# wenhao728/VORTA

Measured on AMD Instinct MI355X. Metric: video_tokens_per_sec (routed-attention denoising step, HunyuanVideo 720p 129f), higher is better.
Workload: dtype fp16

## Files before the change

vorta_amd/_debug.py:

```python
import os

KEYS = ("coreset_kv_order", "fused_text_splits", "sta_merge", "fp8_center_k", "joint_projection", "attn_variant", "no_xcd_remap",
        "sp_staging", "sp_group_streams", "sp_v_wire", "sp_emulate_link_gbps")


def _parse(text: str) -> dict:
    out = {}
    for item in filter(None, (x.strip() for x in text.split(","))):
        key, _, value = item.partition("=")
        if key not in KEYS:
            raise ValueError(f"VORTA_DEBUG: unknown key {key!r} (one of {KEYS})")
        out[key] = value if value else "1"
    return out


FLAGS = _parse(os.environ.get("VORTA_DEBUG", ""))


def flag(key: str, default: str) -> str:
    if key not in KEYS:
        raise KeyError(key)
    return FLAGS.get(key, default)
```

vorta_amd/csrc/attn_common.h:

```cpp
#pragma once
#include <hip/hip_runtime.h>
#include <stdint.h>

#include "vorta_hip.h"
#include "common.h"

namespace vorta_attn {


constexpr int KVB = 64;
constexpr int D = 128;
constexpr int ROWB = D * 2;
constexpr int TILE_BYTES = KVB * ROWB;
constexpr int BUF_BYTES = 2 * TILE_BYTES;

struct Params {
  const char* q; const char* k; const char* v; char* o;
  int64_t q_sh, k_sh, v_sh, o_sh;
  int64_t q_ss, k_ss, v_ss, o_ss;
  const int32_t* head_list; const int32_t* n_heads_dev;
  int n_heads;
  int n_q, q_group_len, q_row_offset, q_valid;
  int n_groups, blocks_per_group;
  const int32_t* q_rows; int64_t q_rows_sh;
  int n_kv, kv_row_offset;
  const int32_t* n_kv_dev; const int32_t* q_valid_dev;
  const int32_t* kv_rows; int64_t kv_rows_sh, kv_rows_sg;
  const int32_t* dup_rows; int64_t dup_rows_sh; int n_dup_pos, n_dup;
  float scale_log2;
  int n_splits, blocks_per_split;
  float* ws_o; float* ws_ml;
  int xcd_remap;
  float defer_log2;
  const int32_t* q_block_table;
  int wg_per_slot;
};

__device__ __forceinline__ void q_block_of(const Params& p, int qb, int rows_per_block, int& grp, int& p0, int& pend) {
  if (p.q_block_table) {
    const int32_t* t = p.q_block_table + 3 * qb;
    grp = t[0]; p0 = t[1]; pend = t[2];
  } else {
    grp = qb / p.blocks_per_group;
    p0 = grp * p.q_group_len + (qb - grp * p.blocks_per_group) * rows_per_block;
    pend = min((grp + 1) * p.q_group_len, p.n_q);
  }
}

__device__ __forceinline__ int live_order(const Params& p, int b, int n, bool remap) {
  if (p.n_heads_dev) n = min(n, max(*p.n_heads_dev, 0) * p.wg_per_slot);
  if (!remap || b >= n) return b;
  const int xcd = b & 7, qd = n >> 3, r = n & 7;
  return (xcd < r ? xcd * (qd + 1) : r * (qd + 1) + (xcd - r) * qd) + (b >> 3);
}

#ifndef VORTA_MAX_SEGMENTS
#define VORTA_MAX_SEGMENTS VORTA_MAX_FUSED_LAUNCHES
#endif
constexpr int MAX_SEGMENTS = VORTA_MAX_SEGMENTS;
template <class PP> __host__ __device__ __forceinline__ Params& base_of(PP& pp) { return pp.p; }
template <class PP> __host__ __device__ __forceinline__ const Params& base_of(const PP& pp) { return pp.p; }
__host__ __device__ __forceinline__ Params& base_of(Params& p) { return p; }
__host__ __device__ __forceinline__ const Params& base_of(const Params& p) { return p; }

template <class PP> struct MultiOf {
  PP seg[MAX_SEGMENTS];
  int start[MAX_SEGMENTS + 1];
  int n;
};

template <class PP>
__device__ __forceinline__ const PP& segment_of(const MultiOf<PP>& mp, int b, int& wg) {
  int s = 0;
#pragma unroll
  for (int i = 1; i < MAX_SEGMENTS; ++i) s += (i < mp.n && b >= mp.start[i]) ? 1 : 0;
  wg = live_order(base_of(mp.seg[s]), b - mp.start[s], mp.start[s + 1] - mp.start[s], true);
  return mp.seg[s];
}

__device__ __forceinline__ float2 out_descale(const Params&, int, int) { return make_float2(1.f, 1.f); }
template <class PP> __device__ __forceinline__ float2 out_descale(const PP& pp, int head, int lane) {
  return *(const float2*)(pp.v_descale + (int64_t)head * pp.v_descale_sh + lane * 2);
}

template <typename T, class PP>
__global__ __launch_bounds__(256) void attn_combine_kernel(const PP pp) {
  const Params& p = base_of(pp);
  const int lane = threadIdx.x & 63;
  const int64_t item = (int64_t)blockIdx.x * 4 + (threadIdx.x >> 6);
  if (item >= (int64_t)p.n_heads * p.n_q) return;
  const int y = (int)(item / p.n_q);
  const int pos = (int)(item - (int64_t)y * p.n_q);
  if (p.n_heads_dev && y >= *p.n_heads_dev) return;
  const int head = p.head_list ? p.head_list[y] : y;
  float m = -1e30f;
  for (int s = 0; s < p.n_splits; ++s) m = fmaxf(m, p.ws_ml[(((int64_t)y * p.n_splits + s) * p.n_q + pos) * 2]);
  float acc0 = 0.f, acc1 = 0.f, l = 0.f;
  for (int s = 0; s < p.n_splits; ++s) {
    const int64_t slot = ((int64_t)y * p.n_splits + s) * p.n_q + pos;
    const float w = __builtin_amdgcn_exp2f(p.ws_ml[slot * 2] - m);
    l += w * p.ws_ml[slot * 2 + 1];
// ... 28 lines not shown

template <typename T, class PP>
int launch_single(void (*kernel)(PP), int block_rows, const PP& pp, hipStream_t st) {
  const Params& p = base_of(pp);
  const int64_t total = (int64_t)p.n_groups * p.blocks_per_group * p.n_heads * p.n_splits;
  if (total <= 0) return VORTA_OK;
  if (total > 0x7fffffff) return VORTA_EINVAL;
  hipLaunchKernelGGL(kernel, dim3((unsigned)total), dim3(block_rows * 2), 0, st, pp);
  const hipError_t e = hipGetLastError();
  if (e != hipSuccess) return vorta_set_hip_error(e);
  return launch_combine<T>(pp, st);
}

template <class F>
int fwd_single(const F& f, const vorta_attn_args* a, void* hip_stream) {
  typename F::PP pp{};
  int block_rows = 0;
  const int rc = f.fill(a, pp, block_rows);
  if (rc != VORTA_OK) return rc;
  if (base_of(pp).n_heads == 0 || base_of(pp).n_groups == 0) return VORTA_OK;
  hipStream_t st = (hipStream_t)hip_stream;
  if (f.out_dtype(*a) == VORTA_BF16) return launch_single<__bf16>(F::template kernel<__bf16>(*a, pp, block_rows), block_rows, pp, st);
  return launch_single<_Float16>(F::template kernel<_Float16>(*a, pp, block_rows), block_rows, pp, st);
}

template <typename T, class PP>
int launch_fused(void (*kernel)(MultiOf<PP>), const MultiOf<PP>& mp, int total, hipStream_t st) {
  hipLaunchKernelGGL(kernel, dim3((unsigned)total), dim3(512), 0, st, mp);
  const hipError_t e = hipGetLastError();
  if (e != hipSuccess) return vorta_set_hip_error(e);
  for (int i = 0; i < mp.n; ++i) {
    const int rc = launch_combine<T>(mp.seg[i], st);
    if (rc != VORTA_OK) return rc;
  }
  return VORTA_OK;
}

template <class F>
int fwd_batch(const F& f, const vorta_attn_args* args, int32_t n, void* hip_stream) {
  if (!args || n < 0 || n > MAX_SEGMENTS) return VORTA_EINVAL;
  MultiOf<typename F::PP> mp{};
  int64_t total = 0;
  int dtype = -1, m = 0;
  for (int i = 0; i < n; ++i) {
    typename F::PP pp{};
    int block_rows = 0;
    const int rc = f.fill(&args[i], pp, block_rows);
    if (rc != VORTA_OK) return rc;
    Params& p = base_of(pp);
    if (p.n_heads == 0 || p.n_groups == 0) continue;
    if (block_rows != 256 || !f.fusable(args[i], pp)) return VORTA_EUNSUPPORTED;
    if (dtype >= 0 && dtype != f.out_dtype(args[i])) return VORTA_EINVAL;
    dtype = f.out_dtype(args[i]);
    p.xcd_remap = 0;
    mp.seg[m] = pp;
    mp.start[m] = (int)total;
    total += (int64_t)p.n_groups * p.blocks_per_group * p.n_heads * p.n_splits;
    if (total > 0x7fffffff) return VORTA_EINVAL;
    ++m;
  }
  if (m == 0) return VORTA_OK;
  for (int i = m; i <= MAX_SEGMENTS; ++i) mp.start[i] = (int)total;
  mp.n = m;
  hipStream_t st = (hipStream_t)hip_stream;
  if (dtype == VORTA_BF16) return launch_fused<__bf16>(F::template multi<__bf16>, mp, (int)total, st);
  return launch_fused<_Float16>(F::template multi<_Float16>, mp, (int)total, st);
}

int fill_params(const vorta_attn_args* a, Params& p, int& block_rows, int in_esize, int v_esize = 0, int k_esize = 0);
int mx_fwd(const vorta_attn_args* a, const vorta_attn_fp8_ext* ext, void* hip_stream);
int mx_fwd_batch(const vorta_attn_args* args, const vorta_attn_fp8_ext* ext, int32_t n, void* hip_stream);

template <typename T> struct MF;
template <> struct MF<__bf16> {
  using v8 = bf16x8; using v4 = bf16x4;
  static __device__ __forceinline__ f32x16 mfma(v8 a, v8 b, f32x16 c) {
    return __builtin_amdgcn_mfma_f32_32x32x16_bf16(a, b, c, 0, 0, 0);
  }
  static __device__ __forceinline__ v4 tr(const char* p) {
    return __builtin_amdgcn_ds_read_tr16_b64_v4bf16((LDS_AS v4*)p);
  }
};
template <> struct MF<_Float16> {
  using v8 = f16x8; using v4 = f16x4;
  static __device__ __forceinline__ f32x16 mfma(v8 a, v8 b, f32x16 c) {
    return __builtin_amdgcn_mfma_f32_32x32x16_f16(a, b, c, 0, 0, 0);
  }
  static __device__ __forceinline__ v4 tr(const char* p) {
    typedef __attribute__((ext_vector_type(4))) __fp16 h4;
    h4 r = __builtin_amdgcn_ds_read_tr16_b64_v4f16((LDS_AS h4*)p);
    return *(v4*)&r;
  }
};

__device__ __forceinline__ float half_max(float x) {
  auto r = __builtin_amdgcn_permlane32_swap(__float_as_uint(x), __float_as_uint(x), false, false);
  return fmaxf(__uint_as_float(r[0]), __uint_as_float(r[1]));
}
__device__ __forceinline__ float half_sum(float x) {
// ... 7 lines not shown
```

vorta_amd/csrc/attn_fwd.hip:

```cpp
#include <hip/hip_runtime.h>
#include <stdint.h>

#include "vorta_hip.h"
#include "common.h"

#include "attn_common.h"
#include "attn_fwd_diag.inc"

namespace {
using namespace vorta_attn;

template <typename T, int NW>
__global__ __launch_bounds__(NW * 64, 2) void attn_fwd_kernel(const Params p) {
  using V8 = typename MF<T>::v8;
  using V4 = typename MF<T>::v4;
  constexpr int NT = NW * 64;
  constexpr int QB = NW * 32;
  constexpr int CH = (KVB * 16) / NT;
  constexpr int ROWSTEP = NT / 16;

  __shared__ __attribute__((aligned(16))) char smem[2 * BUF_BYTES];

  const int wg = live_order(p, blockIdx.x, gridDim.x, p.xcd_remap);
  const int sp = wg % p.n_splits;
  const int rest = wg / p.n_splits;
  const int n_qb = p.n_groups * p.blocks_per_group;
  const int qb = rest % n_qb;
  const int y = rest / n_qb;
  if (p.n_heads_dev && y >= *p.n_heads_dev) return;
  const int head = p.head_list ? p.head_list[y] : y;
  int grp, p0, pend;
  q_block_of(p, qb, QB, grp, p0, pend);

  const int tid = threadIdx.x;
// ... 181 lines not shown
      }
    }
    return;
  }
  if (!row_ok) return;
  const float inv = (my_p < q_valid && l_tot > 0.f) ? 1.f / l_tot : 0.f;
  uint2 packed[16];
#pragma unroll
  for (int dt = 0; dt < 4; ++dt)
#pragma unroll
    for (int rg = 0; rg < 4; ++rg) {
      V4 t;
#pragma unroll
      for (int j = 0; j < 4; ++j) t[j] = (T)(o[dt][4 * rg + j] * inv);
      packed[dt * 4 + rg] = *(uint2*)&t;
    }
  char* obase = p.o + (int64_t)head * p.o_sh + hh * 8;
  auto store_row = [&](int64_t row) {
    char* op = obase + row * p.o_ss;
#pragma unroll
    for (int dt = 0; dt < 4; ++dt)
#pragma unroll
      for (int rg = 0; rg < 4; ++rg) *(uint2*)(op + (32 * dt + 8 * rg) * 2) = packed[dt * 4 + rg];
  };
  store_row(my_row);
  if (p.dup_rows && my_p < p.n_dup_pos) {
    const int32_t* dr = p.dup_rows + (int64_t)y * p.dup_rows_sh + (int64_t)my_p * p.n_dup;
    for (int i = 0; i < p.n_dup; ++i) store_row((int64_t)dr[i]);
  }
}

constexpr int RING = 2;

template <typename T, int NW, bool KVTAB, int NS>
__device__ __forceinline__ void attn_pipe_dma_body(const Params& p, char* __restrict__ smem, const int wg) {
  static_assert(NS == 2, "ring depth");
  TRACE_ENTRY_()
  using V8 = typename MF<T>::v8;
  using V4 = typename MF<T>::v4;
  constexpr int NT = NW * 64;
  constexpr int QB = NW * 32;
  constexpr int CH = (KVB * 16) / NT;
  constexpr int ROWSTEP = NT / 16;
#ifndef VORTA_KPRE
#define VORTA_KPRE 2
#endif
  constexpr int KPRE = (NW == 4 && KVTAB && VORTA_KPRE > 1) ? 1 : VORTA_KPRE;
  const int sp = wg % p.n_splits;
  const int rest = wg / p.n_splits;
  const int n_qb = p.n_groups * p.blocks_per_group;
  const int qb = rest % n_qb;
  const int y = rest / n_qb;
  if (p.n_heads_dev && y >= *p.n_heads_dev) return;
  const int head = p.head_list ? p.head_list[y] : y;
  int grp, p0, pend;
  q_block_of(p, qb, QB, grp, p0, pend);

  const int tid = threadIdx.x;
  const int lane = tid & 63;
  const int wave = __builtin_amdgcn_readfirstlane(tid >> 6);
  const int r32 = lane & 31;
  const int hh = lane >> 5;

  const int n_kv = p.n_kv_dev ? max(1, min(*p.n_kv_dev, p.n_kv)) : p.n_kv;
  const int q_valid = p.q_valid_dev ? min(*p.q_valid_dev, p.q_valid) : p.q_valid;
  const int nblk_total = (n_kv + KVB - 1) / KVB;
  const int blk0 = sp * p.blocks_per_split;
  const int blk1 = min(blk0 + p.blocks_per_split, nblk_total);

  const int wrow0 = p0 + wave * 32;
  const bool wave_active = wrow0 < pend;
  const int my_p = wrow0 + r32;
  const int ld_p = min(my_p, pend - 1);
  const int32_t* q_rows = p.q_rows ? p.q_rows + (int64_t)y * p.q_rows_sh : nullptr;
  const int64_t my_row = q_rows ? (int64_t)q_rows[ld_p] : (int64_t)(p.q_row_offset + ld_p);

  V8 qf[8];
  {
    const char* qp = p.q + (int64_t)head * p.q_sh + my_row * p.q_ss + hh * 16;
#pragma unroll
    for (int ks = 0; ks < 8; ++ks) {
      const V8 raw = *(const V8*)(qp + ks * 32);
#pragma unroll
      for (int i = 0; i < 8; ++i) qf[ks][i] = (T)((float)raw[i] * p.scale_log2);
    }
  }

  const int32_t* kv_rows =
      p.kv_rows ? p.kv_rows + (int64_t)y * p.kv_rows_sh + (int64_t)grp * p.kv_rows_sg : nullptr;
  const char* kbase = p.k + (int64_t)head * p.k_sh + (tid & 15) * 16;
  const char* vbase = p.v + (int64_t)head * p.v_sh + (tid & 15) * 16;
  const int lrow0 = tid >> 4;
  const int lcc = tid & 15;
  const __amdgpu_buffer_rsrc_t k_rsrc = __builtin_amdgcn_make_buffer_rsrc(
      (void*)(p.k + (int64_t)head * p.k_sh), 0, 0x7fffffff, 0x00020000);
  const __amdgpu_buffer_rsrc_t v_rsrc = __builtin_amdgcn_make_buffer_rsrc(
      (void*)(p.v + (int64_t)head * p.v_sh), 0, 0x7fffffff, 0x00020000);
  const int k_ss32 = (int)p.k_ss, v_ss32 = (int)p.v_ss;
// ... 5 lines not shown
    v_col[i] = ((lane & 15) ^ ((row & 3) << 2)) << 4;
  }
  int rowK[CH], rowV[CH];
  int posK[CH];
  unsigned offK[CH], offV[CH];
  const unsigned k_step = (unsigned)(KVB * k_ss32), v_step = (unsigned)(KVB * v_ss32);
#define ROWS_OF(dst_, blk_, clamp_)                                               \
  _Pragma("unroll") for (int i_ = 0; i_ < CH; ++i_) {                             \
    int pos_ = (blk_) * KVB + 4 * (CH * wave + i_) + (lane >> 4);                 \
    if constexpr (clamp_) pos_ = min(pos_, n_kv - 1);                             \
    if constexpr (KVTAB) dst_[i_] = kv_rows[pos_];                                \
    else dst_[i_] = p.kv_row_offset + pos_;                                       \
  }
#define K_OFF(i_) ((int)__umul24((unsigned)rowK[i_], (unsigned)k_ss32) + k_col[i_])
#define V_OFF(i_) ((int)__umul24((unsigned)rowV[i_], (unsigned)v_ss32) + v_col[i_])
#define DMA_K_AT(par_, off_) _Pragma("unroll") for (int i_ = 0; i_ < CH; ++i_) __builtin_amdgcn_raw_ptr_buffer_load_lds( \
      k_rsrc, (LDS_AS void*)(smem + (par_) * TILE_BYTES + (CH * wave + i_) * 1024), 16, (int)(off_), 0, 0, 0);
#define DMA_V_AT(par_, off_) _Pragma("unroll") for (int i_ = 0; i_ < CH; ++i_) __builtin_amdgcn_raw_ptr_buffer_load_lds( \
      v_rsrc, (LDS_AS void*)(smem + (NS + (par_)) * TILE_BYTES + (CH * wave + i_) * 1024), 16, (int)(off_), 0, 0, 0);
#define DMA_K(par_) DMA_K_AT(par_, K_OFF(i_))
#define DMA_V(par_) DMA_V_AT(par_, V_OFF(i_))

  int k_rd[8];
#pragma unroll
  for (int ks = 0; ks < 8; ++ks) k_rd[ks] = r32 * ROWB + (((2 * ks + hh) ^ (r32 & 15)) << 4);
  int v_rd[4];
  {
    const int g = lane >> 4, i16 = lane & 15, q4 = i16 >> 2, pp = i16 & 3;
#pragma unroll
    for (int dt = 0; dt < 4; ++dt)
      v_rd[dt] = NS * TILE_BYTES + (4 * (g >> 1) + q4) * ROWB + ((dt ^ q4) << 6) + 32 * (g & 1) + 8 * pp;
  }

  f32x16 o[4];
#pragma unroll
  for (int dt = 0; dt < 4; ++dt)
#pragma unroll
    for (int i = 0; i < 16; ++i) o[dt][i] = 0.f;
  float m_run = -1e30f, l_run = 0.f;
  const float defer = p.defer_log2;
  f32x16 sA0, sA1, sB0, sB1;
  f32x16 minit;
#pragma unroll
  for (int i = 0; i < 16; ++i) minit[i] = 0.f;
  float mx_cur = -1e30f;

#define QK(d0_, d1_, par_)                                                        \
  {                                                                               \
    _Pragma("unroll") for (int ks_ = 0; ks_ < 8; ++ks_) {                         \
      const V8 k0_ = *(const V8*)(smem + (par_) * TILE_BYTES + k_rd[ks_]);        \
      const V8 k1_ = *(const V8*)(smem + (par_) * TILE_BYTES + k_rd[ks_] + 32 * ROWB); \
      d0_ = MF<T>::mfma(k0_, qf[ks_], ks_ == 0 ? minit : d0_);                    \
      d1_ = MF<T>::mfma(k1_, qf[ks_], ks_ == 0 ? minit : d1_);                    \
    }                                                                             \
  }
#define ROW_MAX(dst_, a_, b_)                                                      \
  {                                                                               \
    float mx_ = a_[0];                                                            \
    _Pragma("unroll") for (int i_ = 1; i_ < 16; ++i_) mx_ = fmaxf(mx_, a_[i_]);   \
    _Pragma("unroll") for (int i_ = 0; i_ < 16; ++i_) mx_ = fmaxf(mx_, b_[i_]);   \
    dst_ = half_max(mx_);                                                         \
  }
#define ROW_MAX_POS(dst_, a_, b_)                                                  \
  {                                                                               \
    int m0_ = max(max(__float_as_int(a_[0]), __float_as_int(a_[1])), __float_as_int(a_[2])); \
    int m1_ = max(max(__float_as_int(b_[0]), __float_as_int(b_[1])), __float_as_int(b_[2])); \
    _Pragma("unroll") for (int i_ = 3; i_ < 15; i_ += 2) {                        \
      m0_ = max(max(m0_, __float_as_int(a_[i_])), __float_as_int(a_[i_ + 1]));    \
      m1_ = max(max(m1_, __float_as_int(b_[i_])), __float_as_int(b_[i_ + 1]));    \
    }                                                                             \
    m0_ = max(max(m0_, __float_as_int(a_[15])), __float_as_int(b_[15]));          \
    m0_ = max(m0_, m1_);                                                          \
    auto r_ = __builtin_amdgcn_permlane32_swap((unsigned)m0_, (unsigned)m0_, false, false); \
    dst_ = __int_as_float(max((int)r_[0], (int)r_[1]));                           \
  }
#define QK_PRE(d0_, d1_, par_)                                                    \
  {                                                                               \
// ... 52 lines not shown
  _Pragma("unroll") for (int g_ = 0; g_ < 16; ++g_) {                             \
    __builtin_amdgcn_sched_group_barrier(0x008, 1, 0);                            \
    __builtin_amdgcn_sched_group_barrier(0x100, 1, 0);                            \
    __builtin_amdgcn_sched_group_barrier(0x400, 2, 0);                            \
    __builtin_amdgcn_sched_group_barrier(0x002, 2, 0);                            \
  }                                                                               \
  _Pragma("unroll") for (int g_ = 0; g_ < 16; ++g_) {                             \
    __builtin_amdgcn_sched_group_barrier(0x008, 1, 0);                            \
    __builtin_amdgcn_sched_group_barrier(0x100, 2, 0);                            \
    __builtin_amdgcn_sched_group_barrier(0x002, 4, 0);                            \
  }
#else
#define SCHED_RECIPE()
#endif
#define STEP(c0_, c1_, n0_, n1_, kcur_, knext_, vfree_, j_, tail_)                \
  {  \
    STAGE_DMA(kcur_, vfree_, j_, tail_)                                           \
    STEP_BODY(c0_, c1_, n0_, n1_, kcur_, knext_, j_, tail_)                       \
    STEP_SYNC()                                                                   \
  }
#define STEP_BODY(c0_, c1_, n0_, n1_, kcur_, knext_, j_, tail_)                   \
  {                                                                               \
    if (wave_active) {                                                            \
      V8 kpre_[KPRE > 0 ? KPRE : 1][2];                                                          \
      _Pragma("unroll") for (int ks_ = 0; ks_ < KPRE; ++ks_) {                    \
        kpre_[ks_][0] = *(const V8*)(smem + (knext_) * TILE_BYTES + k_rd[ks_]);   \
        kpre_[ks_][1] = *(const V8*)(smem + (knext_) * TILE_BYTES + k_rd[ks_] + 32 * ROWB); \
      }                                                                           \
       \
       \
      if ((tail_) && (j_) * KVB + KVB > n_kv) {                                   \
        int h4_ = 4 * hh;  \
        asm volatile("" : "+v"(h4_));                                             \
        _Pragma("unroll") for (int i_ = 0; i_ < 16; ++i_) {                       \
          const int row_ = (i_ & 3) + 8 * (i_ >> 2) + h4_;                        \
          if ((j_) * KVB + row_ >= n_kv) c0_[i_] = -INFINITY;                     \
          if ((j_) * KVB + 32 + row_ >= n_kv) c1_[i_] = -INFINITY;                \
        }                                                                         \
        ROW_MAX(mx_cur, c0_, c1_)                                                 \
      }                                                                           \
       \
       \
       \
      if (!__all(mx_cur <= defer)) {                                              \
        const float g_ = fmaxf(mx_cur, 0.f);                                      \
        RAISE_REF(g_, c0_, c1_)                                                   \
      }                                                                           \
      V8 pb_[4];                                                                  \
      QK_PRE(n0_, n1_, knext_)     \
      float lsum_ = 0.f;                                                          \
      _Pragma("unroll") for (int i_ = 0; i_ < 16; ++i_) {                         \
        c0_[i_] = __builtin_amdgcn_exp2f(c0_[i_]);                                \
        c1_[i_] = __builtin_amdgcn_exp2f(c1_[i_]);                                \
        lsum_ += c0_[i_] + c1_[i_];                                               \
      }                                                                           \
      l_run += lsum_;                                                             \
      _Pragma("unroll") for (int e_ = 0; e_ < 8; ++e_) {                          \
        pb_[0][e_] = (T)c0_[e_];                                                  \
        pb_[1][e_] = (T)c0_[8 + e_];                                              \
        pb_[2][e_] = (T)c1_[e_];                                                  \
        pb_[3][e_] = (T)c1_[8 + e_];                                              \
      }                                                                           \
      _Pragma("unroll") for (int dt_ = 0; dt_ < 4; ++dt_) {                       \
        _Pragma("unroll") for (int kg_ = 0; kg_ < 4; ++kg_) {                     \
          const V4 lo_ = MF<T>::tr(smem + (kcur_) * TILE_BYTES + v_rd[dt_] + (16 * kg_) * ROWB); \
          const V4 hi_ = MF<T>::tr(smem + (kcur_) * TILE_BYTES + v_rd[dt_] + (16 * kg_ + 8) * ROWB); \
          V8 vf_;                                                                 \
          _Pragma("unroll") for (int e_ = 0; e_ < 4; ++e_) { vf_[e_] = lo_[e_]; vf_[4 + e_] = hi_[e_]; } \
          o[dt_] = MF<T>::mfma(vf_, pb_[kg_], o[dt_]);                            \
        }                                                                         \
      }                                                                           \
      ROW_MAX_POS(mx_cur, n0_, n1_)  \
      SCHED_RECIPE()                                                              \
    }                                                                             \
  }

  if (blk0 < blk1) {
    ROWS_OF(rowK, blk0, true)
    _Pragma("unroll") for (int i_ = 0; i_ < CH; ++i_) rowV[i_] = rowK[i_];
    DMA_K(0)
    DMA_V(0)
    ROWS_OF(rowK, blk0 + 1, true)
    DMA_K(1)
    _Pragma("unroll") for (int i_ = 0; i_ < CH; ++i_) rowV[i_] = rowK[i_];
    ROWS_OF(rowK, blk0 + NS, true)
    _Pragma("unroll") for (int i_ = 0; i_ < CH; ++i_) posK[i_] = (blk0 + NS) * KVB + 4 * (CH * wave + i_) + (lane >> 4);
    if constexpr (!KVTAB) {
      _Pragma("unroll") for (int i_ = 0; i_ < CH; ++i_) { offK[i_] = (unsigned)K_OFF(i_); offV[i_] = (unsigned)V_OFF(i_); }
    }
    __syncthreads();
    if (wave_active) {
      QK(sA0, sA1, 0)
      if (blk0 * KVB + KVB > n_kv) {
#pragma unroll
        for (int i = 0; i < 16; ++i) {
          const int row = (i & 3) + 8 * (i >> 2) + 4 * hh;
          if (blk0 * KVB + row >= n_kv) sA0[i] = -INFINITY;
          if (blk0 * KVB + 32 + row >= n_kv) sA1[i] = -INFINITY;
        }
      }
      ROW_MAX(mx_cur, sA0, sA1)
      m_run = mx_cur;
#pragma unroll
      for (int i = 0; i < 16; ++i) { sA0[i] -= m_run; sA1[i] -= m_run; minit[i] = -m_run; }
      asm volatile("" : "+v"(minit));
      mx_cur = 0.f;
    }
    __syncthreads();
  }
  const int blk_whole = min(blk1, n_kv / KVB - (KVTAB ? NS + 1 : NS));
  int blk = blk0;
  for (; blk + 1 < blk_whole; blk += 2) {
    STEP(sA0, sA1, sB0, sB1, 0, 1, 1, blk, false)
    STEP(sB0, sB1, sA0, sA1, 1, 0, 0, blk + 1, false)
  }
  if constexpr (!KVTAB) {
    if (blk > blk0 && blk < blk1) {
      ROWS_OF(rowV, blk + 1, true)
      ROWS_OF(rowK, blk + NS, true)
      _Pragma("unroll") for (int i_ = 0; i_ < CH; ++i_) posK[i_] = (blk + NS) * KVB + 4 * (CH * wave + i_) + (lane >> 4);
    }
  }
  for (; blk < blk1; blk += 2) {
    STEP(sA0, sA1, sB0, sB1, 0, 1, 1, blk, true)
    if (blk + 1 >= blk1) break;
    STEP(sB0, sB1, sA0, sA1, 1, 0, 0, blk + 1, true)
  }
#undef QK
#undef QK_PRE
#undef ROW_MAX
#undef ROW_MAX_POS
#undef RAISE_REF
#undef STEP
#undef STEP_BODY
#undef STAGE_DMA
#undef STEP_SYNC
#undef ROWS_OF
#undef DMA_K
#undef DMA_V
#undef DMA_K_AT
#undef DMA_V_AT
#undef K_OFF
#undef V_OFF

  TRACE_FLUSH_()
  if (!wave_active) return;
  int tid_e = threadIdx.x;
  asm volatile("" : "+v"(tid_e));
  const int hh_e = (tid_e >> 5) & 1;
  const int e_p = wrow0 + (tid_e & 31);
  const bool e_ok = e_p < pend;
  const int64_t e_row = q_rows ? (int64_t)q_rows[min(e_p, pend - 1)] : (int64_t)(p.q_row_offset + min(e_p, pend - 1));
  const float l_tot = half_sum(l_run);
  if (p.n_splits > 1) {
    if (e_ok) {
      const int64_t slot = ((int64_t)y * p.n_splits + sp) * p.n_q + e_p;
      float* wo = p.ws_o + slot * D;
#pragma unroll
      for (int dt = 0; dt < 4; ++dt)
#pragma unroll
        for (int rg = 0; rg < 4; ++rg) {
          f32x4 v = {o[dt][4 * rg], o[dt][4 * rg + 1], o[dt][4 * rg + 2], o[dt][4 * rg + 3]};
          *(f32x4*)(wo + 32 * dt + 8 * rg + 4 * hh_e) = v;
        }
      if (hh_e == 0) {
        p.ws_ml[slot * 2] = m_run;
        p.ws_ml[slot * 2 + 1] = l_tot;
      }
    }
    return;
  }
  if (!e_ok) return;
  const float inv = (e_p < q_valid && l_tot > 0.f) ? 1.f / l_tot : 0.f;
  uint2 packed[16];
#pragma unroll
  for (int dt = 0; dt < 4; ++dt)
#pragma unroll
    for (int rg = 0; rg < 4; ++rg) {
      V4 t;
#pragma unroll
      for (int j = 0; j < 4; ++j) t[j] = (T)(o[dt][4 * rg + j] * inv);
      packed[dt * 4 + rg] = *(uint2*)&t;
    }
  char* obase = p.o + (int64_t)head * p.o_sh + hh_e * 8;
  auto store_row = [&](int64_t row) {
    char* op = obase + row * p.o_ss;
#pragma unroll
    for (int dt = 0; dt < 4; ++dt)
#pragma unroll
      for (int rg = 0; rg < 4; ++rg) *(uint2*)(op + (32 * dt + 8 * rg) * 2) = packed[dt * 4 + rg];
  };
  store_row(e_row);
  if (p.dup_rows && e_p < p.n_dup_pos) {
    const int32_t* dr = p.dup_rows + (int64_t)y * p.dup_rows_sh + (int64_t)e_p * p.n_dup;
    for (int i = 0; i < p.n_dup; ++i) store_row((int64_t)dr[i]);
  }
}


template <typename T, int NW, bool KVTAB>
__global__ __launch_bounds__(NW * 64, 2) void attn_fwd_pipe_kernel(const Params p) {
#if defined(__HIP_DEVICE_COMPILE__)
  constexpr int NS = RING;
  __shared__ __attribute__((aligned(16))) char smem[2 * NS * TILE_BYTES];
  const int wg = live_order(p, blockIdx.x, gridDim.x, p.xcd_remap);
  attn_pipe_dma_body<T, NW, KVTAB, NS>(p, smem, wg);
#endif
}


template <typename T>
__global__ __launch_bounds__(512, 2) void attn_fwd_multi_kernel(const MultiOf<Params> mp) {
#if defined(__HIP_DEVICE_COMPILE__)
  __shared__ __attribute__((aligned(16))) char smem[2 * RING * TILE_BYTES];
  int wg;
  const Params& p = segment_of(mp, blockIdx.x, wg);
  if (p.kv_rows) attn_pipe_dma_body<T, 8, true, RING>(p, smem, wg);
  else attn_pipe_dma_body<T, 8, false, RING>(p, smem, wg);
#endif
}

}

int vorta_attn::fill_params(const vorta_attn_args* a, Params& p, int& block_rows, int in_esize, int v_esize, int k_esize) {
  if (v_esize == 0) v_esize = in_esize;
  if (k_esize == 0) k_esize = in_esize;
  if (!a || a->struct_size != sizeof(vorta_attn_args)) return VORTA_EINVAL;
  if (in_esize == 2 ? (a->dtype != VORTA_BF16 && a->dtype != VORTA_FP16) : a->dtype != VORTA_FP8E4M3) return VORTA_EUNSUPPORTED;
  if (a->head_dim != D) return VORTA_EUNSUPPORTED;
  if (a->n_heads < 0 || a->n_q < 0 || a->n_kv < 0) return VORTA_EINVAL;
  if (a->n_heads == 0 || a->n_q == 0) { block_rows = 0; p.n_groups = 0; p.blocks_per_group = 0; p.n_heads = 0; return VORTA_OK; }
  if (a->n_kv == 0) return VORTA_EINVAL;
  if (!a->q.ptr || !a->k.ptr || !a->v.ptr || !a->o.ptr) return VORTA_EINVAL;
  const vorta_tensor* ts[4] = {&a->q, &a->k, &a->v, &a->o};
  for (int i = 0; i < 4; ++i) {
    const vorta_tensor* t = ts[i];
    const int al = 16 / (i == 0 ? in_esize : i == 1 ? k_esize : i == 2 ? v_esize : 2);
    if (((uintptr_t)t->ptr & 15) || (t->stride_s % al) || (t->stride_h % al) || t->stride_s < D) return VORTA_EINVAL;
  }
  if (a->n_splits < 1 || a->n_splits > 1024) return VORTA_EINVAL;
  if (!(a->scale > 0.f)) return VORTA_EINVAL;
  if (a->n_splits > 1 && (!a->ws_o || !a->ws_ml)) return VORTA_EINVAL;
  if (a->q_group_len < 0 || a->q_valid < 0) return VORTA_EINVAL;
  if (a->dup_rows && (a->n_dup < 0 || a->n_dup_pos < 0 || a->n_dup_pos > a->n_q)) return VORTA_EINVAL;
  if (a->block_rows != 0 && a->block_rows != 128 && a->block_rows != 256) return VORTA_EINVAL;
  if (a->variant < 0 || a->variant > 2) return VORTA_EINVAL;
  if (a->variant != 1 && (a->k.stride_s * k_esize >= (1 << 24) || a->v.stride_s * v_esize >= (1 << 24))) return VORTA_EUNSUPPORTED;
  if (a->variant != 1 && !a->kv_rows) {
    const int64_t last = (int64_t)a->kv_row_offset + a->n_kv;
    const int64_t ks = a->k.stride_s * k_esize, vs = a->v.stride_s * v_esize;
    const int64_t ss = ks > vs ? ks : vs;
// ... 4 lines not shown
  p.q_ss = a->q.stride_s * in_esize; p.k_ss = a->k.stride_s * k_esize; p.v_ss = a->v.stride_s * v_esize; p.o_ss = a->o.stride_s * 2;
  p.head_list = a->head_list; p.n_heads_dev = a->n_heads_dev; p.n_heads = a->n_heads;
  p.n_q = a->n_q; p.q_group_len = a->q_group_len > 0 ? a->q_group_len : a->n_q;
  p.q_row_offset = a->q_row_offset; p.q_valid = a->q_valid;
  p.q_rows = a->q_rows; p.q_rows_sh = a->q_rows_stride_h;
  p.n_kv = a->n_kv; p.kv_row_offset = a->kv_row_offset;
  p.n_kv_dev = a->n_kv_dev; p.q_valid_dev = a->q_valid_dev;
  p.kv_rows = a->kv_rows; p.kv_rows_sh = a->kv_rows_stride_h; p.kv_rows_sg = a->kv_rows_stride_g;
  p.dup_rows = a->dup_rows; p.dup_rows_sh = a->dup_rows_stride_h; p.n_dup_pos = a->n_dup_pos; p.n_dup = a->n_dup;
  p.scale_log2 = a->scale * 1.4426950408889634f;
  p.n_splits = a->n_splits; p.ws_o = a->ws_o; p.ws_ml = a->ws_ml;
  p.xcd_remap = (a->reserved & 1) ? 0 : 1;
  p.defer_log2 = (a->reserved & 4) ? 0.f : 6.f;
  p.n_groups = (p.n_q + p.q_group_len - 1) / p.q_group_len;
  block_rows = a->block_rows;
  if (block_rows == 0) {
    const int g = p.q_group_len;
    const int64_t pad256 = ((g + 255) / 256) * 256, pad128 = ((g + 127) / 128) * 128;
    block_rows = (pad256 * 100 > pad128 * 106) ? 128 : 256;
  }
  p.blocks_per_group = (p.q_group_len + block_rows - 1) / block_rows;
  p.q_block_table = a->q_block_table;
  if (a->q_block_table) {
    if (a->n_q_blocks <= 0 || (a->block_rows != 128 && a->block_rows != 256)) return VORTA_EINVAL;
    p.n_groups = a->n_q_blocks;
    p.blocks_per_group = 1;
  }
  const int nblk = (p.n_kv + KVB - 1) / KVB;
  p.blocks_per_split = (nblk + p.n_splits - 1) / p.n_splits;
  p.wg_per_slot = p.n_groups * p.blocks_per_group * p.n_splits;
  return VORTA_OK;
}

namespace {
using namespace vorta_attn;

struct Family16 {
  using PP = Params;
  int fill(const vorta_attn_args* a, Params& p, int& block_rows) const { return fill_params(a, p, block_rows, 2); }
  bool fusable(const vorta_attn_args& a, const Params&) const { return a.variant != 1; }
  int out_dtype(const vorta_attn_args& a) const { return a.dtype; }
  template <typename T> static constexpr auto multi = attn_fwd_multi_kernel<T>;
  template <typename T> static auto kernel(const vorta_attn_args& a, const Params& p, int block_rows) {
    if (a.variant == 1) return block_rows == 256 ? attn_fwd_kernel<T, 8> : attn_fwd_kernel<T, 4>;
    if (block_rows == 256) return p.kv_rows ? attn_fwd_pipe_kernel<T, 8, true> : attn_fwd_pipe_kernel<T, 8, false>;
    return p.kv_rows ? attn_fwd_pipe_kernel<T, 4, true> : attn_fwd_pipe_kernel<T, 4, false>;
  }
};
}

extern "C" int vorta_attn_workspace_bytes(const vorta_attn_args* a, uint64_t* ws_o_bytes, uint64_t* ws_ml_bytes) {
  if (!a || a->struct_size != sizeof(vorta_attn_args) || !ws_o_bytes || !ws_ml_bytes) return VORTA_EINVAL;
  if (a->n_splits <= 1) { *ws_o_bytes = 0; *ws_ml_bytes = 0; return VORTA_OK; }
  const uint64_t slots = (uint64_t)a->n_heads * (uint64_t)a->n_splits * (uint64_t)a->n_q;
  *ws_o_bytes = slots * D * sizeof(float);
  *ws_ml_bytes = slots * 2 * sizeof(float);
  return VORTA_OK;
}

extern "C" int vorta_attn_plan(const vorta_attn_args* a, int32_t* block_rows_out, int64_t* n_workgroups_out,
                               int32_t* kernel_id_out) {
  Params p{};
  int block_rows = 0;
  int rc = vorta_attn::fill_params(a, p, block_rows, (a && a->dtype == VORTA_FP8E4M3) ? 1 : 2);
  if (rc != VORTA_OK) return rc;
  if (block_rows_out) *block_rows_out = block_rows;
  if (kernel_id_out) {
    const bool pipe = a->variant != 1;
    *kernel_id_out = (block_rows == 256 ? 8 : 4) * 16 + (pipe ? 1 : 0) + ((pipe && a->kv_rows) ? 2 : 0);
  }
  if (n_workgroups_out) *n_workgroups_out = (int64_t)p.n_groups * p.blocks_per_group * p.n_heads * (p.n_heads ? p.n_splits : 0);
  return VORTA_OK;
}

// ... 6 lines not shown
```

vorta_amd/ops.py:

```python
from __future__ import annotations

import ctypes as C
import math
from typing import NamedTuple, Optional, Sequence, Tuple

import torch

from . import _C

_DT = {torch.bfloat16: _C.VORTA_BF16, torch.float16: _C.VORTA_FP16}
FP8_STORAGE = torch.uint8


class Timeline:

    def __init__(self):
        self.records = []

    def summary(self):
        torch.cuda.synchronize()
        out = {}
        for tag, br, nwg, flops, e0, e1 in self.records:
            d = out.setdefault((tag, br), dict(launches=0, ms=0.0, flops=0.0, workgroups=0))
            d["launches"] += 1
            d["ms"] += e0.elapsed_time(e1)
            d["flops"] += flops
            d["workgroups"] += nwg
        return out


_timeline: Optional[Timeline] = None
from ._debug import flag as _debug_flag
DEFAULT_VARIANT = int(_debug_flag("attn_variant", "0"))
NO_XCD_REMAP = int(_debug_flag("no_xcd_remap", "0"))


def set_timeline(t: Optional[Timeline]):
    global _timeline
    _timeline = t


def _stream() -> int:
    return torch.cuda.current_stream().cuda_stream


def _require_gpu(*ts: torch.Tensor):
    for t in ts:
        if t is not None and not t.is_cuda:
            raise _C.VortaHipError("vorta_amd ops need tensors on an MI355X (cuda) device; there is no CPU path")


def _tensor(t: torch.Tensor) -> _C.Tensor:
    if t.dim() != 3 or t.stride(2) != 1:
        raise ValueError(f"expected a (H,S,D) view with contiguous D, got shape {tuple(t.shape)} strides {t.stride()}")
    return _C.Tensor(t.data_ptr(), t.stride(0), t.stride(1))


def _ptr(t: Optional[torch.Tensor], dtype=torch.int32):
    if t is None:
        return None
    if t.dtype != dtype or not t.is_contiguous():
        raise ValueError(f"index tables must be contiguous {dtype}")
    return t.data_ptr()


def fold_heads(x: torch.Tensor) -> torch.Tensor:
    if x.dim() == 3:
# ... 105 lines not shown
            raise ValueError("query groups need kv_rows_stride_g (one key list per group)")
        elif kv_rows.dim() not in (1, 2) or kv_rows.shape[-1] < n_kv or (kv_rows.dim() == 2 and kv_rows.shape[0] < n_heads):
            raise ValueError(f"kv_rows {tuple(kv_rows.shape)} does not cover n_kv = {n_kv} keys for {n_heads} head slots "
                             f"(1-D: shared by all heads; 2-D: one row per head slot)")
    if dup_rows is not None and (dup_rows.dim() not in (2, 3) or (dup_rows.dim() == 3 and dup_rows.shape[0] < n_heads)
                                 or dup_rows.shape[-2] < (n_dup_pos or dup_rows.shape[-2])):
        raise ValueError(f"dup_rows {tuple(dup_rows.shape)} does not cover {n_dup_pos} positions for {n_heads} head slots")
    a.q_rows = _ptr(q_rows)
    a.q_rows_stride_h = q_rows.stride(0) if (q_rows is not None and q_rows.dim() == 2) else 0
    a.n_kv, a.kv_row_offset = n_kv, kv_row_offset
    a.kv_rows = _ptr(kv_rows)
    if kv_rows is not None and kv_rows_stride_g == 0 and kv_rows.dim() == 2:
        a.kv_rows_stride_h = kv_rows.stride(0)
    a.kv_rows_stride_g = kv_rows_stride_g
    a.dup_rows = _ptr(dup_rows)
    if dup_rows is not None:
        if dup_rows.dim() == 3:
            a.dup_rows_stride_h = dup_rows.stride(0)
        a.n_dup = dup_rows.shape[-1]
        a.n_dup_pos = n_dup_pos if n_dup_pos else dup_rows.shape[-2]
    a.scale = (1.0 / math.sqrt(q.shape[-1])) if scale is None else scale
    a.block_rows = block_rows
    a.n_splits = n_splits
    a.n_kv_dev, a.q_valid_dev = _ptr(n_kv_dev), _ptr(q_valid_dev)
    a.variant = 0 if (fp8 or mixed or i8) else (variant or DEFAULT_VARIANT)
    if a.variant != 1:
        for t in (k, v):
            esz = t.element_size()
            if t.shape[1] >= (1 << 24) or t.shape[1] * t.stride(1) * esz > 0x7fffffff or t.stride(1) * esz >= (1 << 24):
                if fp8 or mixed or i8:
                    raise ValueError("fp8 attention addresses K/V rows with 32-bit offsets: a head must fit a 2 GiB window")
                a.variant = 1
    a.reserved = NO_XCD_REMAP
    if q_block_table is not None:
        a.q_block_table, a.n_q_blocks = _ptr(q_block_table), q_block_table.shape[0]
    ws = None
    if n_splits > 1:
        so, sm = C.c_uint64(), C.c_uint64()
        _C.check(_C.lib().vorta_attn_workspace_bytes(C.byref(a), C.byref(so), C.byref(sm)), "vorta_attn_workspace_bytes")
        ws = (torch.empty(so.value // 4, dtype=torch.float32, device=q.device),
              torch.empty(sm.value // 4, dtype=torch.float32, device=q.device))
        a.ws_o, a.ws_ml = ws[0].data_ptr(), ws[1].data_ptr()
    return a, ws


class _Family(NamedTuple):
    one: str
    batch: str
    kernel: str
    multi: str


_FAMILIES = {
    "16": _Family("vorta_attn_fwd", "vorta_attn_fwd_batch", "attn_fwd_pipe_kernel<{t},{nw},{tab}>", "attn_fwd_multi_kernel<{t}>"),
    "fp8": _Family("vorta_attn_fwd_fp8", "vorta_attn_fwd_batch_fp8", "attn8_kernel<{t},{nw},{tab},{lmfma}>", "attn8_multi_kernel<{t}>"),
    "mx": _Family("vorta_attn_fwd_fp8", "vorta_attn_fwd_batch_fp8", "attn_mx_kernel<{t},{nw},{tab}>", "attn_mx_multi_kernel<{t}>"),
    "i8": _Family("vorta_attn_fwd_i8", "vorta_attn_fwd_batch_i8", "attn_i8_kernel<{t},{nw},{tab}>", "attn_i8_multi_kernel<{t}>"),
}


def _ext(a) -> tuple:
    return () if a._ext is None else (C.byref(a._ext),)


def _launch_one(a):
    name = a._family.one
# ... 718 lines not shown
```

Baseline: 27790.

## Make fused attention kernel persistent with per-XCD atomic work queues

The fused multi-segment attention kernel now launches at most one workgroup per CU, and each workgroup loops pulling work items from per-XCD atomic counters, stealing from other XCDs when its own queue runs dry. The next item is prefetched partway through the current one so the atomic's latency overlaps compute. The aim is to cut launch and tail imbalance and to keep XCD-local L2 reuse. In exchange it adds atomics, a counter ring with a memset per launch, and uniform-load and masking tweaks. Because the grid is capped at the CU count, only one workgroup runs per CU even though launch bounds allow two, which may reduce latency hiding.

Measured after the change: 28770, median of 6. 3.5% higher.

```diff
diff --git a/vorta_amd/_debug.py b/vorta_amd/_debug.py
--- a/vorta_amd/_debug.py
+++ b/vorta_amd/_debug.py
@@ -1,7 +1,7 @@
 import os
 
 KEYS = ("coreset_kv_order", "fused_text_splits", "sta_merge", "fp8_center_k", "joint_projection", "attn_variant", "no_xcd_remap",
-        "sp_staging", "sp_group_streams", "sp_v_wire", "sp_emulate_link_gbps")
+        "sp_staging", "sp_group_streams", "sp_v_wire", "sp_emulate_link_gbps", "persistent_wgs")
 
 
 def _parse(text: str) -> dict:
diff --git a/vorta_amd/csrc/attn_common.h b/vorta_amd/csrc/attn_common.h
--- a/vorta_amd/csrc/attn_common.h
+++ b/vorta_amd/csrc/attn_common.h
@@ -1,6 +1,8 @@
 #pragma once
 #include <hip/hip_runtime.h>
 #include <stdint.h>
+
+#include <type_traits>
 
 #include "vorta_hip.h"
 #include "common.h"
@@ -36,10 +38,17 @@
   int wg_per_slot;
 };
 
-__device__ __forceinline__ void q_block_of(const Params& p, int qb, int rows_per_block, int& grp, int& p0, int& pend) {
+template <bool OPAQUE>
+__device__ __forceinline__ int32_t load_uniform(const int32_t* ptr, int vz = 0) {
+  if constexpr (OPAQUE) return __builtin_amdgcn_readfirstlane(ptr[vz]);
+  else return *ptr;
+}
+
+template <bool OPAQUE = false>
+__device__ __forceinline__ void q_block_of(const Params& p, int qb, int rows_per_block, int& grp, int& p0, int& pend, int vz = 0) {
   if (p.q_block_table) {
     const int32_t* t = p.q_block_table + 3 * qb;
-    grp = t[0]; p0 = t[1]; pend = t[2];
+    grp = load_uniform<OPAQUE>(t, vz); p0 = load_uniform<OPAQUE>(t + 1, vz); pend = load_uniform<OPAQUE>(t + 2, vz);
   } else {
     grp = qb / p.blocks_per_group;
     p0 = grp * p.q_group_len + (qb - grp * p.blocks_per_group) * rows_per_block;
@@ -67,6 +76,11 @@
   PP seg[MAX_SEGMENTS];
   int start[MAX_SEGMENTS + 1];
   int n;
+};
+
+template <class PP> struct PersistOf {
+  MultiOf<PP> m;
+  uint32_t* counters;
 };
 
 template <class PP>
@@ -161,6 +175,29 @@
   for (int i = 0; i < mp.n; ++i) {
     const int rc = launch_combine<T>(mp.seg[i], st);
     if (rc != VORTA_OK) return rc;
+  }
+  return VORTA_OK;
+}
+
+template <class F, class = void> struct is_persistent : std::false_type {};
+template <class F> struct is_persistent<F, std::void_t<decltype(F::persistent)>> : std::bool_constant<F::persistent> {};
+
+int persist_acquire(hipStream_t st, uint32_t** counters, int* n_cu);
+
+template <typename T, class PP>
+int launch_persistent(void (*kernel)(PersistOf<PP>), const MultiOf<PP>& mp, int total, int cap, hipStream_t st) {
+  PersistOf<PP> pm{mp, nullptr};
+  int n_cu = 0;
+  const int rc = persist_acquire(st, &pm.counters, &n_cu);
+  if (rc != VORTA_OK) return rc;
+  int grid = total < n_cu ? total : n_cu;
+  if (cap > 0 && cap < grid) grid = cap;
+  hipLaunchKernelGGL(kernel, dim3((unsigned)grid), dim3(512), 0, st, pm);
+  const hipError_t e = hipGetLastError();
+  if (e != hipSuccess) return vorta_set_hip_error(e);
+  for (int i = 0; i < mp.n; ++i) {
+    const int rc2 = launch_combine<T>(mp.seg[i], st);
+    if (rc2 != VORTA_OK) return rc2;
   }
   return VORTA_OK;
 }
@@ -192,8 +229,14 @@
   for (int i = m; i <= MAX_SEGMENTS; ++i) mp.start[i] = (int)total;
   mp.n = m;
   hipStream_t st = (hipStream_t)hip_stream;
-  if (dtype == VORTA_BF16) return launch_fused<__bf16>(F::template multi<__bf16>, mp, (int)total, st);
-  return launch_fused<_Float16>(F::template multi<_Float16>, mp, (int)total, st);
+  if constexpr (is_persistent<F>::value) {
+    const int cap = (args[0].reserved >> 16) & 0x7fff;
+    if (dtype == VORTA_BF16) return launch_persistent<__bf16>(F::template multi<__bf16>, mp, (int)total, cap, st);
+    return launch_persistent<_Float16>(F::template multi<_Float16>, mp, (int)total, cap, st);
+  } else {
+    if (dtype == VORTA_BF16) return launch_fused<__bf16>(F::template multi<__bf16>, mp, (int)total, st);
+    return launch_fused<_Float16>(F::template multi<_Float16>, mp, (int)total, st);
+  }
 }
 
 int fill_params(const vorta_attn_args* a, Params& p, int& block_rows, int in_esize, int v_esize = 0, int k_esize = 0);
diff --git a/vorta_amd/csrc/attn_fwd.hip b/vorta_amd/csrc/attn_fwd.hip
--- a/vorta_amd/csrc/attn_fwd.hip
+++ b/vorta_amd/csrc/attn_fwd.hip
@@ -1,5 +1,8 @@
 #include <hip/hip_runtime.h>
 #include <stdint.h>
+
+#include <mutex>
+#include <utility>
 
 #include "vorta_hip.h"
 #include "common.h"
@@ -247,8 +250,62 @@
 
 constexpr int RING = 2;
 
-template <typename T, int NW, bool KVTAB, int NS>
-__device__ __forceinline__ void attn_pipe_dma_body(const Params& p, char* __restrict__ smem, const int wg) {
+template <int ROW>
+__device__ __forceinline__ float mask_row(float x, int lim, float ninf) {
+  asm("v_cmp_ge_i32 vcc, %2, %1\n\tv_cndmask_b32 %0, %0, %3, vcc" : "+v"(x) : "v"(lim), "n"(ROW), "v"(ninf) : "vcc");
+  return x;
+}
+template <int... I>
+__device__ __forceinline__ void mask_rows(f32x16& a, f32x16& b, int lim, std::integer_sequence<int, I...>) {
+  float ninf = -INFINITY;
+  asm volatile("" : "+v"(ninf));
+  ((a[I] = mask_row<(I & 3) + 8 * (I >> 2)>(a[I], lim, ninf), b[I] = mask_row<32 + (I & 3) + 8 * (I >> 2)>(b[I], lim, ninf)), ...);
+}
+
+template <bool RESTRICT> struct ParamsRefOf { typedef const Params& type; };
+template <> struct ParamsRefOf<true> { typedef const Params& __restrict__ type; };
+template <bool RESTRICT> using ParamsRef = typename ParamsRefOf<RESTRICT>::type;
+
+struct PersistShared {
+  int seg_n[MAX_SEGMENTS];
+  int qlen[8];
+  int item[2];
+  uint32_t* counters;
+  int xcd;
+};
+
+__device__ __forceinline__ void persist_pull(const PersistShared& sh, int* out) {
+  uint32_t* counters = sh.counters;
+  const int xcd = sh.xcd;
+  int q = -1, v = 0;
+#pragma unroll 1
+  for (int t = 0; t < 8; ++t) {
+    const int x = (xcd + t) & 7;
+    const int len = sh.qlen[x];
+    if (len <= 0) continue;
+    const uint32_t got = __hip_atomic_fetch_add(counters + x, 1u, __ATOMIC_RELAXED, __HIP_MEMORY_SCOPE_AGENT);
+    if (got < (uint32_t)len) { q = x; v = (int)got; break; }
+  }
+  out[0] = q;
+  out[1] = v;
+}
+
+__device__ __forceinline__ int item_lane() {
+  int lane;
+  asm volatile("v_mbcnt_lo_u32_b32 %0, -1, 0\n\tv_mbcnt_hi_u32_b32 %0, -1, %0" : "=v"(lane));
+  return lane;
+}
+
+template <typename T, int NW, bool KVTAB, int NS, bool ITEMS = false>
+__device__ __forceinline__ void attn_pipe_dma_body(ParamsRef<NW == 8> p, char* __restrict__ smem, const int wg,
+                                                   const int item_wave = 0, const int item_state = 0) {
+#define ITEM_HOOK()                                                               \
+  if constexpr (ITEMS) {                                                          \
+    if (item_wave * 64 + item_lane() == 0) {                                      \
+      PersistShared& sh_ = *(PersistShared*)(smem + item_state);                  \
+      persist_pull(sh_, sh_.item);                                                \
+    }                                                                             \
+  }
   static_assert(NS == 2, "ring depth");
   TRACE_ENTRY_()
   using V8 = typename MF<T>::v8;
@@ -266,19 +323,23 @@
   const int n_qb = p.n_groups * p.blocks_per_group;
   const int qb = rest % n_qb;
   const int y = rest / n_qb;
-  if (p.n_heads_dev && y >= *p.n_heads_dev) return;
-  const int head = p.head_list ? p.head_list[y] : y;
+  int vz = 0;
+  if constexpr (ITEMS) asm volatile("" : "+v"(vz));
+  if (p.n_heads_dev && y >= load_uniform<ITEMS>(p.n_heads_dev, vz)) { ITEM_HOOK() return; }
+  const int head = p.head_list ? load_uniform<ITEMS>(p.head_list + y, vz) : y;
   int grp, p0, pend;
-  q_block_of(p, qb, QB, grp, p0, pend);
-
-  const int tid = threadIdx.x;
+  q_block_of<ITEMS>(p, qb, QB, grp, p0, pend, vz);
+
+  int tid_ = ITEMS ? item_wave * 64 + item_lane() : (int)threadIdx.x;
+  if constexpr (ITEMS) asm volatile("" : "+v"(tid_));
+  const int tid = tid_;
   const int lane = tid & 63;
   const int wave = __builtin_amdgcn_readfirstlane(tid >> 6);
   const int r32 = lane & 31;
   const int hh = lane >> 5;
 
-  const int n_kv = p.n_kv_dev ? max(1, min(*p.n_kv_dev, p.n_kv)) : p.n_kv;
-  const int q_valid = p.q_valid_dev ? min(*p.q_valid_dev, p.q_valid) : p.q_valid;
+  const int n_kv = p.n_kv_dev ? max(1, min(load_uniform<ITEMS>(p.n_kv_dev, vz), p.n_kv)) : p.n_kv;
+  const int q_valid = p.q_valid_dev ? min(load_uniform<ITEMS>(p.q_valid_dev, vz), p.q_valid) : p.q_valid;
   const int nblk_total = (n_kv + KVB - 1) / KVB;
   const int blk0 = sp * p.blocks_per_split;
   const int blk1 = min(blk0 + p.blocks_per_split, nblk_total);
@@ -350,17 +411,19 @@
       v_rd[dt] = NS * TILE_BYTES + (4 * (g >> 1) + q4) * ROWB + ((dt ^ q4) << 6) + 32 * (g & 1) + 8 * pp;
   }
 
+  float zero = 0.f;
+  if constexpr (ITEMS) asm volatile("" : "+v"(zero));
   f32x16 o[4];
 #pragma unroll
   for (int dt = 0; dt < 4; ++dt)
 #pragma unroll
-    for (int i = 0; i < 16; ++i) o[dt][i] = 0.f;
+    for (int i = 0; i < 16; ++i) o[dt][i] = zero;
   float m_run = -1e30f, l_run = 0.f;
   const float defer = p.defer_log2;
   f32x16 sA0, sA1, sB0, sB1;
   f32x16 minit;
 #pragma unroll
-  for (int i = 0; i < 16; ++i) minit[i] = 0.f;
+  for (int i = 0; i < 16; ++i) minit[i] = zero;
   float mx_cur = -1e30f;
 
 #define QK(d0_, d1_, par_)                                                        \
@@ -479,10 +542,14 @@
       if ((tail_) && (j_) * KVB + KVB > n_kv) {                                   \
         int h4_ = 4 * hh;  \
         asm volatile("" : "+v"(h4_));                                             \
-        _Pragma("unroll") for (int i_ = 0; i_ < 16; ++i_) {                       \
-          const int row_ = (i_ & 3) + 8 * (i_ >> 2) + h4_;                        \
-          if ((j_) * KVB + row_ >= n_kv) c0_[i_] = -INFINITY;                     \
-          if ((j_) * KVB + 32 + row_ >= n_kv) c1_[i_] = -INFINITY;                \
+        if constexpr (ITEMS) {                                                    \
+          mask_rows(c0_, c1_, n_kv - (j_) * KVB - h4_, std::make_integer_sequence<int, 16>{}); \
+        } else {                                                                  \
+          _Pragma("unroll") for (int i_ = 0; i_ < 16; ++i_) {                     \
+            const int row_ = (i_ & 3) + 8 * (i_ >> 2) + h4_;                      \
+            if ((j_) * KVB + row_ >= n_kv) c0_[i_] = -INFINITY;                   \
+            if ((j_) * KVB + 32 + row_ >= n_kv) c1_[i_] = -INFINITY;              \
+          }                                                                       \
         }                                                                         \
         ROW_MAX(mx_cur, c0_, c1_)                                                 \
       }                                                                           \
@@ -535,15 +602,20 @@
     if constexpr (!KVTAB) {
       _Pragma("unroll") for (int i_ = 0; i_ < CH; ++i_) { offK[i_] = (unsigned)K_OFF(i_); offV[i_] = (unsigned)V_OFF(i_); }
     }
+    ITEM_HOOK()
     __syncthreads();
     if (wave_active) {
       QK(sA0, sA1, 0)
       if (blk0 * KVB + KVB > n_kv) {
-#pragma unroll
-        for (int i = 0; i < 16; ++i) {
-          const int row = (i & 3) + 8 * (i >> 2) + 4 * hh;
-          if (blk0 * KVB + row >= n_kv) sA0[i] = -INFINITY;
-          if (blk0 * KVB + 32 + row >= n_kv) sA1[i] = -INFINITY;
+        if constexpr (ITEMS) {
+          mask_rows(sA0, sA1, n_kv - blk0 * KVB - 4 * hh, std::make_integer_sequence<int, 16>{});
+        } else {
+#pragma unroll
+          for (int i = 0; i < 16; ++i) {
+            const int row = (i & 3) + 8 * (i >> 2) + 4 * hh;
+            if (blk0 * KVB + row >= n_kv) sA0[i] = -INFINITY;
+            if (blk0 * KVB + 32 + row >= n_kv) sA1[i] = -INFINITY;
+          }
         }
       }
       ROW_MAX(mx_cur, sA0, sA1)
@@ -554,9 +626,12 @@
       mx_cur = 0.f;
     }
     __syncthreads();
+  } else {
+    ITEM_HOOK()
   }
   const int blk_whole = min(blk1, n_kv / KVB - (KVTAB ? NS + 1 : NS));
   int blk = blk0;
+  if constexpr (ITEMS) __builtin_amdgcn_s_waitcnt(0);
   for (; blk + 1 < blk_whole; blk += 2) {
     STEP(sA0, sA1, sB0, sB1, 0, 1, 1, blk, false)
     STEP(sB0, sB1, sA0, sA1, 1, 0, 0, blk + 1, false)
@@ -573,6 +648,7 @@
     if (blk + 1 >= blk1) break;
     STEP(sB0, sB1, sA0, sA1, 1, 0, 0, blk + 1, true)
   }
+#undef ITEM_HOOK
 #undef QK
 #undef QK_PRE
 #undef ROW_MAX
@@ -592,7 +668,7 @@
 
   TRACE_FLUSH_()
   if (!wave_active) return;
-  int tid_e = threadIdx.x;
+  int tid_e = ITEMS ? item_wave * 64 + item_lane() : (int)threadIdx.x;
   asm volatile("" : "+v"(tid_e));
   const int hh_e = (tid_e >> 5) & 1;
   const int e_p = wrow0 + (tid_e & 31);
@@ -655,15 +731,71 @@
 #endif
 }
 
-
 template <typename T>
-__global__ __launch_bounds__(512, 2) void attn_fwd_multi_kernel(const MultiOf<Params> mp) {
+__global__ __launch_bounds__(512, 2) void attn_fwd_multi_kernel(const PersistOf<Params> pm) {
 #if defined(__HIP_DEVICE_COMPILE__)
-  __shared__ __attribute__((aligned(16))) char smem[2 * RING * TILE_BYTES];
-  int wg;
-  const Params& p = segment_of(mp, blockIdx.x, wg);
-  if (p.kv_rows) attn_pipe_dma_body<T, 8, true, RING>(p, smem, wg);
-  else attn_pipe_dma_body<T, 8, false, RING>(p, smem, wg);
+  __shared__ __attribute__((aligned(16))) char smem[2 * RING * TILE_BYTES + sizeof(PersistShared)];
+  PersistShared& sh0 = *(PersistShared*)(smem + 2 * RING * TILE_BYTES);
+  const int wave = __builtin_amdgcn_readfirstlane(threadIdx.x >> 6);
+  {
+    PersistShared& sh = sh0;
+    const MultiOf<Params>& mp = pm.m;
+    if (threadIdx.x == 0) {
+      sh.counters = pm.counters;
+      sh.xcd = (int)__builtin_amdgcn_s_getreg((20 << 0) | (0 << 6) | (31 << 11)) & 7;
+    }
+    int len = 0;
+#pragma unroll
+    for (int i = 0; i < MAX_SEGMENTS; ++i) {
+      int n = 0;
+      if (i < mp.n) {
+        const Params& p = mp.seg[i];
+        n = mp.start[i + 1] - mp.start[i];
+        if (p.n_heads_dev) n = min(n, max(*p.n_heads_dev, 0) * p.wg_per_slot);
+      }
+      if (threadIdx.x == 0) sh.seg_n[i] = n;
+      len += (n >> 3) + ((int)(threadIdx.x & 7) < (n & 7) ? 1 : 0);
+    }
+    if (threadIdx.x < 8) sh.qlen[threadIdx.x] = len;
+    __syncthreads();
+    if (threadIdx.x == 0) persist_pull(sh, sh.item);
+    __syncthreads();
+  }
+  for (;;) {
+    int z = 0;
+    asm volatile("" : "+s"(z));
+    const MultiOf<Params>& mp = (&pm.m)[z];
+    PersistShared& sh = (&sh0)[z];
+    const int q = __builtin_amdgcn_readfirstlane(sh.item[0]);
+    if (q < 0) break;
+    int j = __builtin_amdgcn_readfirstlane(sh.item[1]);
+    asm volatile("s_waitcnt lgkmcnt(0)\n\ts_barrier" ::: "memory");
+    int s = 0, n = 0;
+    bool found = false;
+#pragma unroll
+    for (int i = 0; i < MAX_SEGMENTS; ++i) {
+      const int ni = __builtin_amdgcn_readfirstlane(sh.seg_n[i]);
+      const int li = (ni >> 3) + (q < (ni & 7) ? 1 : 0);
+      if (!found) {
+        if (j < li) { found = true; s = i; n = ni; }
+        else j -= li;
+      }
+    }
+    const int qd = n >> 3, r = n & 7;
+    const int wg = (q < r ? q * (qd + 1) : r * (qd + 1) + (q - r) * qd) + j;
+    const Params& p = mp.seg[s];
+    const int state = 2 * RING * TILE_BYTES + z * (int)sizeof(PersistShared);
+    if (p.kv_rows) attn_pipe_dma_body<T, 8, true, RING, true>(p, smem, wg, wave, state);
+    else attn_pipe_dma_body<T, 8, false, RING, true>(p, smem, wg, wave, state);
+    asm volatile("s_waitcnt lgkmcnt(0)\n\ts_barrier" ::: "memory");
+  }
+  if (threadIdx.x == 0) {
+    uint32_t* counters = sh0.counters;
+    if (__hip_atomic_fetch_add(counters + 8, 1u, __ATOMIC_ACQ_REL, __HIP_MEMORY_SCOPE_AGENT) == gridDim.x - 1) {
+#pragma unroll
+      for (int i = 0; i < 9; ++i) __hip_atomic_store(counters + i, 0u, __ATOMIC_RELAXED, __HIP_MEMORY_SCOPE_AGENT);
+    }
+  }
 #endif
 }
 
@@ -734,6 +866,58 @@
   return VORTA_OK;
 }
 
+int vorta_attn::persist_acquire(hipStream_t st, uint32_t** counters, int* n_cu) {
+  constexpr int PERSIST_RING = 4096, SLOT_WORDS = 16, MAX_DEVICES = 64;
+  struct Ring { uint32_t* buf = nullptr; int n_cu = 0; uint32_t next = 0; uint32_t* cap = nullptr; int cap_left = 0; };
+  static Ring rings[MAX_DEVICES];
+  static std::mutex mu;
+  int dev = 0;
+  hipError_t e = hipGetDevice(&dev);
+  if (e != hipSuccess) return vorta_set_hip_error(e);
+  if (dev < 0 || dev >= MAX_DEVICES) return VORTA_EUNSUPPORTED;
+  hipStreamCaptureStatus capturing = hipStreamCaptureStatusNone;
+  e = hipStreamIsCapturing(st, &capturing);
+  if (e != hipSuccess) return vorta_set_hip_error(e);
+  auto chunk = [](uint32_t** out) {
+    const size_t bytes = (size_t)PERSIST_RING * SLOT_WORDS * sizeof(uint32_t);
+    hipStreamCaptureMode mode = hipStreamCaptureModeRelaxed;
+    (void)hipThreadExchangeStreamCaptureMode(&mode);
+    void* buf = nullptr;
+    hipError_t e = hipMalloc(&buf, bytes);
+    if (e == hipSuccess) e = hipMemset(buf, 0, bytes);
+    if (e == hipSuccess) e = hipStreamSynchronize(nullptr);
+    (void)hipThreadExchangeStreamCaptureMode(&mode);
+    if (e != hipSuccess && buf) (void)hipFree(buf);
+    *out = e == hipSuccess ? (uint32_t*)buf : nullptr;
+    return e;
+  };
+  std::lock_guard<std::mutex> lock(mu);
+  Ring& r = rings[dev];
+  if (!r.n_cu) {
+    e = hipDeviceGetAttribute(&r.n_cu, hipDeviceAttributeMultiprocessorCount, dev);
+    if (e != hipSuccess) return vorta_set_hip_error(e);
+  }
+  *n_cu = r.n_cu;
+  if (!r.buf) {
+    e = chunk(&r.buf);
+    if (e == hipSuccess) e = chunk(&r.cap);
+    if (e != hipSuccess) return vorta_set_hip_error(e);
+    r.cap_left = PERSIST_RING;
+  }
+  if (capturing != hipStreamCaptureStatusNone) {
+    if (r.cap_left == 0) {
+      e = chunk(&r.cap);
+      if (e != hipSuccess) return vorta_set_hip_error(e);
+      r.cap_left = PERSIST_RING;
+    }
+    *counters = r.cap + (size_t)(PERSIST_RING - r.cap_left--) * SLOT_WORDS;
+    return VORTA_OK;
+  }
+  *counters = r.buf + (size_t)(r.next++ % PERSIST_RING) * SLOT_WORDS;
+  e = hipMemsetAsync(*counters, 0, 9 * sizeof(uint32_t), st);
+  return e == hipSuccess ? VORTA_OK : vorta_set_hip_error(e);
+}
+
 namespace {
 using namespace vorta_attn;
 
@@ -742,6 +926,7 @@
   int fill(const vorta_attn_args* a, Params& p, int& block_rows) const { return fill_params(a, p, block_rows, 2); }
   bool fusable(const vorta_attn_args& a, const Params&) const { return a.variant != 1; }
   int out_dtype(const vorta_attn_args& a) const { return a.dtype; }
+  static constexpr bool persistent = true;
   template <typename T> static constexpr auto multi = attn_fwd_multi_kernel<T>;
   template <typename T> static auto kernel(const vorta_attn_args& a, const Params& p, int block_rows) {
     if (a.variant == 1) return block_rows == 256 ? attn_fwd_kernel<T, 8> : attn_fwd_kernel<T, 4>;
diff --git a/vorta_amd/ops.py b/vorta_amd/ops.py
--- a/vorta_amd/ops.py
+++ b/vorta_amd/ops.py
@@ -33,6 +33,7 @@
 from ._debug import flag as _debug_flag
 DEFAULT_VARIANT = int(_debug_flag("attn_variant", "0"))
 NO_XCD_REMAP = int(_debug_flag("no_xcd_remap", "0"))
+PERSISTENT_WGS = int(_debug_flag("persistent_wgs", "0"))
 
 
 def set_timeline(t: Optional[Timeline]):
@@ -204,6 +205,8 @@
                     raise ValueError("fp8 attention addresses K/V rows with 32-bit offsets: a head must fit a 2 GiB window")
                 a.variant = 1
     a.reserved = NO_XCD_REMAP
+    if not (fp8 or mixed or i8):
+        a.reserved |= min(max(PERSISTENT_WGS, 0), 0x7fff) << 16
     if q_block_table is not None:
         a.q_block_table, a.n_q_blocks = _ptr(q_block_table), q_block_table.shape[0]
     ws = None
```
